# visionworkbench/visionworkbench

Measured on AMD Instinct MI355X. Metric: disparity Mpix/s, 4096x4096 pair, 7x7 SAD, +-64-px search, higher is better.
Workload: dtype u8

## Files before the change

### visionworkbench_amd/csrc/bm_sad_u8.hip

```cpp
#include <climits>
#include <cstdlib>
#include <type_traits>

#include "vwgpu_internal.h"
#include "u8_tile.h"

#ifdef VWGPU_TILE_STAMPS
__device__ unsigned long long* g_sad_stamps = nullptr;
extern "C" int vwgpu_debug_set_sad_stamps(void* d_buf) {
  unsigned long long* p = static_cast<unsigned long long*>(d_buf);
  return hipMemcpyToSymbol(HIP_SYMBOL(g_sad_stamps), &p, sizeof p) == hipSuccess ? 0 : -3;
}
#define VWGPU_STAMP(k) do { if (g_sad_stamps && tid == 0) g_sad_stamps[(size_t)wg * 16 + (k)] = wall_clock64(); } while (0)
#else
#define VWGPU_STAMP(k) do { } while (0)
#endif

namespace {

using namespace vwgpu_u8;
typedef uint32_t u32;
typedef uint64_t u64;
typedef unsigned short u16x2 __attribute__((ext_vector_type(2)));

__device__ __forceinline__ u32 pk_sub_u16(u32 a, u32 b) {
  return __builtin_bit_cast(u32, (u16x2)(__builtin_bit_cast(u16x2, a) - __builtin_bit_cast(u16x2, b)));
}
__device__ __forceinline__ u32 pk_max_u16(u32 a, u32 b) {
  return __builtin_bit_cast(u32, __builtin_elementwise_max(__builtin_bit_cast(u16x2, a), __builtin_bit_cast(u16x2, b)));
}
__device__ __forceinline__ u32 pk_min_u16(u32 a, u32 b) {
  return __builtin_bit_cast(u32, __builtin_elementwise_min(__builtin_bit_cast(u16x2, a), __builtin_bit_cast(u16x2, b)));
}
__device__ __forceinline__ void umin3_acc(u32& k, u32 a, u32 b) {
  asm volatile("v_min3_u32 %0, %0, %1, %2" : "+v"(k) : "v"(a), "v"(b));
}

template <int W>
__device__ __forceinline__ void key_sub(u32& key, u32 a, u32 b) {
  if (W == 0)
    asm volatile("v_sub_u16_sdwa %0, %1, %2 dst_sel:WORD_1 dst_unused:UNUSED_PRESERVE src0_sel:WORD_0 src1_sel:WORD_0"
                 : "+v"(key) : "v"(a), "v"(b));
  else
    asm volatile("v_sub_u16_sdwa %0, %1, %2 dst_sel:WORD_1 dst_unused:UNUSED_PRESERVE src0_sel:WORD_1 src1_sel:WORD_1"
                 : "+v"(key) : "v"(a), "v"(b));
}

template <int KX, int KY, int TY, int WV = 0>
struct Cfg {
  static constexpr int NW = (KX + 3) / 4;
  static constexpr int EW = NW <= 2 ? 2 : 4;
  static constexpr int WAVES = WV ? WV : (NW <= 2 ? 4 : 2);
  static constexpr int THREADS = WAVES * 64;
  static constexpr int TWB = WAVES * 256;
  static constexpr int NR = TY + KY - 1;
  static constexpr int LBW = TWB / 4 + NW + 1;
  static constexpr u32 LAST_MASK = (KX % 4 == 0) ? 0xffffffffu : ((1u << (8 * (KX % 4))) - 1u);
};

__device__ __forceinline__ void divmod_small(int idx, int d, float inv, int& quo, int& rem) {
  int qq = (int)(((float)idx + 0.5f) * inv);
  int rr = idx - qq * d;
  if (rr < 0) { --qq; rr += d; }
  if (rr >= d) { ++qq; rr -= d; }
  quo = qq; rem = rr;
}

__device__ __forceinline__ bool sad_second_on_cu(unsigned block, int first_round) {
  return (int)(block >> 3) >= (first_round >> 4);
}

__host__ __device__ constexpr size_t ent_words(int nr, int ne, int ew, int gr, int ty, int pt) {
  const size_t ent = (size_t)nr * ne * ew;
  const size_t merge = gr > 1 ? (size_t)(gr - 1) * (ty / gr) * 4 * pt + (size_t)gr * pt : 0;
  const size_t ob = (size_t)gr * (pt / 64) * 768;
  return ent > merge ? (ent > ob ? ent : ob) : (merge > ob ? merge : ob);
}

template <int KX, int KY, int TY, int GR, int WV = 0, bool EM = true, bool STREAM = false>
__global__ void __launch_bounds__((GR * (Cfg<KX, KY, TY, WV>::THREADS)), (GR > 1 ? 1 : (TY <= 8 && KX <= 8 ? 3 : 2)))
bm_sad_u8_kernel(const float* __restrict__ L, ptrdiff_t ls, int lw, int lh,
                 const float* __restrict__ R, ptrdiff_t rs, int rcw, int rch,
                 int sx, int sy, int ne, int32_t* __restrict__ out, ptrdiff_t os, int ow, int oh,
                 int* __restrict__ flag_set, int* __restrict__ flag_clear,
                 int gxt, int ntiles, int last_round, int first_round, int stagger_ticks) {
  typedef Cfg<KX, KY, TY, WV> C;
  constexpr bool SPLIT = GR > 1;
  static_assert(!(STREAM && SPLIT), "streaming output stores: one-group kernels only");
  constexpr int NW = C::NW, EW = C::EW, NR = C::NR;
  constexpr int NRP = EM ? (NR | 1) : NR;
  extern __shared__ __attribute__((aligned(16))) u32 lds[];
  u32* ent = lds;
  const int bpitch = ne + NW + 1;
  u32* base = lds + ent_words(NRP, ne, EW, GR, TY, C::THREADS);
  u32* item_ctr = base + (size_t)NR * bpitch;

  constexpr int PT = C::THREADS;
  constexpr int NT = GR * PT;
  const int tid = threadIdx.x;
  const int grp = SPLIT ? __builtin_amdgcn_readfirstlane(tid / PT) : 0;
  const int ltid = SPLIT ? tid % PT : tid;
  const int pair_id = __builtin_amdgcn_readfirstlane(ltid >> 6);
  const int per_xcd = gridDim.x >> 3;
  const int wg = (int)(blockIdx.x & 7) * per_xcd + (int)(blockIdx.x >> 3);
  if (wg >= ntiles) return;
  const int x0 = (wg % gxt) * C::TWB;
  const int y0 = (wg / gxt) * TY;
  const int q = x0 + 4 * ltid;
  u32 bad_acc = 0;
  if (wg == 0 && tid == 0) *flag_clear = 0;
#ifdef VWGPU_TILE_STAMPS
  if (g_sad_stamps && tid == 0) {
    unsigned hw, xcc;
    asm volatile("s_getreg_b32 %0, hwreg(HW_REG_HW_ID)" : "=s"(hw));
    asm volatile("s_getreg_b32 %0, hwreg(HW_REG_XCC_ID)" : "=s"(xcc));
    unsigned long long* rec = g_sad_stamps + (size_t)wg * 16;
    rec[0] = wall_clock64(); rec[1] = clock64(); rec[2] = ((unsigned long long)xcc << 32) | hw;
  }
#endif

  if (!SPLIT && (int)blockIdx.x < first_round && sad_second_on_cu(blockIdx.x, first_round)) {
    if (tid < 64) {
      const u64 t_start = wall_clock64();
      for (int it = 0; it < 512 && wall_clock64() - t_start < (u64)stagger_ticks; ++it) __builtin_amdgcn_s_sleep(8);
    }
    __syncthreads();
  }
  stage_u8_rows<NR>(L, ls, lw, lh, x0, y0, C::LBW, C::LBW, ent, tid, NT, bad_acc);
  stage_u8_rows<NR>(R, rs, rcw, rch, x0, y0, bpitch, bpitch, base, tid, NT, bad_acc);
  __syncthreads();
  u64 win[NR][NW];
#pragma unroll
  for (int r = 0; r < NR; ++r) {
    u32 a[NW + 1];
#pragma unroll
    for (int n = 0; n <= NW; ++n) a[n] = ent[r * C::LBW + ltid + n];
#pragma unroll
    for (int n = 0; n < NW; ++n) win[r][n] = (u64)a[n] | ((u64)a[n + 1] << 32);
  }

  VWGPU_STAMP(3);
  u32 K[TY][4];
  u32 MN[TY][2], MX[TY][2];
#pragma unroll
  for (int y = 0; y < TY; ++y) K[y][0] = K[y][1] = K[y][2] = K[y][3] = 0xffffffffu;
  u32 eq_rows = (1u << TY) - 1u;
  int eq_checks = 0;
  constexpr int NPROBE = 4;
  const u32 zero = 0;

  const bool late = !SPLIT && (int)blockIdx.x >= last_round;
  if (!SPLIT) { if (late) __builtin_amdgcn_s_setprio(2); else __builtin_amdgcn_s_setprio(3); }
  typedef std::true_type T;
  typedef std::false_type F;

  auto sweep = [&](auto max_tag) __attribute__((always_inline)) {
    constexpr bool MAXSWEEP = decltype(max_tag)::value;
    for (int dy = 0; dy < sy; ++dy) {
      __syncthreads();
      if (dy > 0 || (MAXSWEEP && sy > 1)) stage_u8_rows<NR>(R, rs, rcw, rch, x0, y0 + dy, bpitch, bpitch, base, tid, NT, bad_acc);
      for (int t = 0; t < 4; ++t) {
        const int a_last = (sx + 2 - t) >> 2;
        __syncthreads();
        if (!MAXSWEEP && !SPLIT && dy == 0 && late) {
          if (t == 2) __builtin_amdgcn_s_setprio(1);
          else if (t == 3) __builtin_amdgcn_s_setprio(0);
        }
        {
          auto build = [&](int r, int m) __attribute__((always_inline)) {
            const u32* bp = base + (size_t)r * bpitch + m;
            u32 b[NW + 1];
#pragma unroll
            for (int n = 0; n <= NW; ++n) b[n] = bp[n];
            u32 w[EW];
#pragma unroll
            for (int n = 0; n < EW; ++n) w[n] = 0;
#pragma unroll
            for (int n = 0; n < NW; ++n) w[n] = __builtin_amdgcn_alignbyte(b[n + 1], b[n], t);
            w[NW - 1] &= C::LAST_MASK;
            u32* e = ent + (EM ? (size_t)m * NRP + r : (size_t)r * ne + m) * EW;
            if (EW == 2) *reinterpret_cast<uint2*>(e) = make_uint2(w[0], w[1]);
            else *reinterpret_cast<uint4*>(e) = make_uint4(w[0], w[1], w[2 % EW], w[3 % EW]);
          };
#pragma unroll 4
          for (int r = grp; r < NR; r += NT / PT) build(r, ltid);
          const int rem = ne - PT, total = NR * rem;
          const float inv = 1.0f / (float)rem;
          for (int idx = tid; idx < total; idx += NT) {
            int r, m;
            divmod_small(idx, rem, inv, r, m);
            build(r, PT + m);
          }
          if (SPLIT && tid < PT / 64) item_ctr[tid] = 0u;
        }
        __syncthreads();

        auto step = [&](int a, auto masked_tag, auto pair_tag, auto probe_tag) __attribute__((always_inline)) {
          constexpr bool MASKED = decltype(masked_tag)::value;
          constexpr bool PAIR = decltype(pair_tag)::value;
          constexpr bool PROBE = decltype(probe_tag)::value;
          const int jbase = 4 * a + t;
          const int ibase = dy * sx + jbase;
          u32 kinA[4], kinB[4];
          u32 orA[2] = {0u, 0u};
#pragma unroll
          for (int i = 0; i < 4; ++i) {
            kinA[i] = (u32)(ibase - i) & 0xffffu;
            kinB[i] = (u32)(ibase + 4 - i) & 0xffffu;
            if (MASKED) {
              const int d = jbase - i;
              if (d < 0 || d >= sx) orA[i >> 1] |= (i & 1) ? 0xffff0000u : 0x0000ffffu;
            }
          }
          const u32* ep = ent + (size_t)(ltid + a) * (EM ? NRP * EW : EW);
          u64 accA = 0, accB = 0;
          u64 PA[NR], PB[NR];
          constexpr int PF = 4;
          u32 wa[NR][EW], wb[NR][EW];
          auto fetch = [&](int r) __attribute__((always_inline)) {
            const u32* e = ep + (EM ? (size_t)r * EW : (size_t)r * ne * EW);
            constexpr int NX = EM ? NRP * EW : EW;
            if (EW == 2) {
              const uint2 v = *reinterpret_cast<const uint2*>(e);
              wa[r][0] = v.x; wa[r][1] = v.y;
              if (PAIR) { const uint2 u = *reinterpret_cast<const uint2*>(e + NX); wb[r][0] = u.x; wb[r][1] = u.y; }
            } else {
              const uint4 v = *reinterpret_cast<const uint4*>(e);
              wa[r][0] = v.x; wa[r][1] = v.y; wa[r][2 % EW] = v.z; wa[r][3 % EW] = v.w;
              if (PAIR) { const uint4 u = *reinterpret_cast<const uint4*>(e + NX); wb[r][0] = u.x; wb[r][1] = u.y; wb[r][2 % EW] = u.z; wb[r][3 % EW] = u.w; }
            }
          };
#pragma unroll
          for (int r = 0; r < PF && r < NR; ++r) fetch(r);
#pragma unroll
          for (int r = 0; r < NR; ++r) {
            if (r + PF < NR) fetch(r + PF);
#pragma unroll
            for (int n = 0; n < NW; ++n) {
              accA = __builtin_amdgcn_qsad_pk_u16_u8(win[r][n], wa[r][n], accA);
              if (PAIR) accB = __builtin_amdgcn_qsad_pk_u16_u8(win[r][n], wb[r][n], accB);
            }
            PA[r] = accA;
            if (PAIR) PB[r] = accB;
            if (r >= KY - 1) {
              const int y = r - (KY - 1);
              const int ro = (r >= KY) ? r - KY : 0;
              const u32 nA0 = (u32)PA[r], nA1 = (u32)(PA[r] >> 32);
              const u32 oA0 = (r >= KY) ? (u32)PA[ro] : zero;
              const u32 oA1 = (r >= KY) ? (u32)(PA[ro] >> 32) : zero;
              if (MAXSWEEP) {
                const u32 sA0 = pk_sub_u16(nA0, oA0), sA1 = pk_sub_u16(nA1, oA1);
                MN[y][0] = pk_min_u16(MN[y][0], MASKED ? (sA0 | orA[0]) : sA0);
                MN[y][1] = pk_min_u16(MN[y][1], MASKED ? (sA1 | orA[1]) : sA1);
                MX[y][0] = pk_max_u16(MX[y][0], MASKED ? (sA0 & ~orA[0]) : sA0);
                MX[y][1] = pk_max_u16(MX[y][1], MASKED ? (sA1 & ~orA[1]) : sA1);
                if (PAIR) {
                  const u32 nB0 = (u32)PB[r], nB1 = (u32)(PB[r] >> 32);
                  const u32 oB0 = (r >= KY) ? (u32)PB[ro] : zero;
                  const u32 oB1 = (r >= KY) ? (u32)(PB[ro] >> 32) : zero;
                  const u32 sB0 = pk_sub_u16(nB0, oB0), sB1 = pk_sub_u16(nB1, oB1);
                  MN[y][0] = pk_min_u16(MN[y][0], sB0);
                  MN[y][1] = pk_min_u16(MN[y][1], sB1);
                  MX[y][0] = pk_max_u16(MX[y][0], sB0);
                  MX[y][1] = pk_max_u16(MX[y][1], sB1);
                }
              } else {
                key_sub<0>(kinA[0], nA0, oA0); key_sub<1>(kinA[1], nA0, oA0);
                key_sub<0>(kinA[2], nA1, oA1); key_sub<1>(kinA[3], nA1, oA1);
                if (PAIR) {
                  const u32 nB0 = (u32)PB[r], nB1 = (u32)(PB[r] >> 32);
                  const u32 oB0 = (r >= KY) ? (u32)PB[ro] : zero;
                  const u32 oB1 = (r >= KY) ? (u32)(PB[ro] >> 32) : zero;
                  key_sub<0>(kinB[0], nB0, oB0); key_sub<1>(kinB[1], nB0, oB0);
                  key_sub<0>(kinB[2], nB1, oB1); key_sub<1>(kinB[3], nB1, oB1);
                  if (PROBE) {
                    u32 x[4];
#pragma unroll
                    for (int i = 0; i < 4; ++i) {
                      asm volatile("v_xor_b32 %0, %1, %2" : "=v"(x[i]) : "v"(kinA[i]), "v"(kinB[i]));
                      x[i] = (q + i < ow) ? x[i] : 0xffffffffu;
                    }
                    const u32 m01 = x[0] < x[1] ? x[0] : x[1], m23 = x[2] < x[3] ? x[2] : x[3];
                    if ((m01 < m23 ? m01 : m23) >> 16) eq_rows &= ~(1u << y);
                  }
                  umin3_acc(K[y][0], kinA[0], kinB[0]);
                  umin3_acc(K[y][1], kinA[1], kinB[1]);
                  umin3_acc(K[y][2], kinA[2], kinB[2]);
                  umin3_acc(K[y][3], kinA[3], kinB[3]);
                } else {
                  const u32 kA0 = (MASKED && (orA[0] & 0x0000ffffu)) ? 0xffffffffu : kinA[0];
                  const u32 kA1 = (MASKED && (orA[0] & 0xffff0000u)) ? 0xffffffffu : kinA[1];
                  const u32 kA2 = (MASKED && (orA[1] & 0x0000ffffu)) ? 0xffffffffu : kinA[2];
                  const u32 kA3 = (MASKED && (orA[1] & 0xffff0000u)) ? 0xffffffffu : kinA[3];
                  umin3_acc(K[y][0], kA0, kA0);
                  umin3_acc(K[y][1], kA1, kA1);
                  umin3_acc(K[y][2], kA2, kA2);
                  umin3_acc(K[y][3], kA3, kA3);
                }
              }
            }
          }
        };

        int a_lo = (t >= 3) ? 0 : 1;
        int a_hi = (sx - 1 - t >= 0) ? ((sx - 1 - t) >> 2) + 1 : 0;
        if (a_hi > a_last + 1) a_hi = a_last + 1;
        if (a_lo > a_hi) a_lo = a_hi;
        const int n1 = a_lo;
        const int npair = (a_hi - n1) > 0 ? (a_hi - n1) >> 1 : 0;
        int nprobe = 0;
        if (!MAXSWEEP && dy == 0 && t == 0) nprobe = npair < NPROBE - eq_checks ? npair : NPROBE - eq_checks;
        const int a4 = n1 + 2 * npair;
        const int n4 = a_last - a4 + 1 > 0 ? a_last - a4 + 1 : 0;
        const int nitems = n1 + npair + n4;
        int seq = 0;
        auto next_item = [&]() __attribute__((always_inline)) -> int {
          if (MAXSWEEP) return grp == 0 ? seq++ : 0x7fffffff;
          if (!SPLIT) return seq++;
          int lane, v = 0;
          asm volatile("v_mbcnt_lo_u32_b32 %0, -1, 0\n\tv_mbcnt_hi_u32_b32 %0, -1, %0" : "=v"(lane));
          if (lane == 0) v = (int)atomicAdd(&item_ctr[pair_id], 1u);
          return __builtin_amdgcn_readfirstlane(v);
        };
        int i = next_item();
        for (; i < n1; i = next_item()) step(i, T{}, F{}, F{});
        for (; i < n1 + nprobe; i = next_item()) step(n1 + 2 * (i - n1), F{}, T{}, T{});
        for (; i < n1 + npair; i = next_item()) step(n1 + 2 * (i - n1), F{}, T{}, F{});
        for (; i < nitems; i = next_item()) step(a4 + (i - n1 - npair), T{}, F{}, F{});
        eq_checks += nprobe;
        if (!MAXSWEEP && dy == 0) VWGPU_STAMP(4 + t);
      }
    }
  };
  sweep(F{});
  if (!SPLIT) __builtin_amdgcn_s_setprio(3);

  if (bad_acc != 0u) atomicOr(flag_set, 1);
  constexpr int RG = TY / GR;
  static_assert(TY % GR == 0, "rows per group");
  auto row_mine = [&](int y) __attribute__((always_inline)) -> bool { return !SPLIT || (y / RG == grp); };
  if (SPLIT) {
    u32* xk = ent;
    u32* xe = ent + (size_t)(GR - 1) * RG * 4 * PT;
    u32 eq_all = eq_rows;
#pragma unroll
    for (int d = 0; d < GR; ++d) {
      __syncthreads();
      if (grp != d) {
        const int slot = grp < d ? grp : grp - 1;
#pragma unroll
        for (int y = 0; y < RG; ++y)
#pragma unroll
          for (int s2 = 0; s2 < 4; ++s2) xk[((slot * RG + y) * 4 + s2) * PT + ltid] = K[d * RG + y][s2];
      }
      if (d == 0) xe[grp * PT + ltid] = eq_rows;
      __syncthreads();
      if (grp == d) {
#pragma unroll
        for (int slot = 0; slot < GR - 1; ++slot)
#pragma unroll
          for (int y = 0; y < RG; ++y)
#pragma unroll
            for (int s2 = 0; s2 < 4; ++s2) {
              const u32 o = xk[((slot * RG + y) * 4 + s2) * PT + ltid];
              K[d * RG + y][s2] = o < K[d * RG + y][s2] ? o : K[d * RG + y][s2];
            }
      }
      if (d == 0) {
#pragma unroll
        for (int g2 = 0; g2 < GR; ++g2) eq_all &= xe[g2 * PT + ltid];
      }
    }
    eq_rows = eq_all;
  }
  u32 cand = eq_checks < NPROBE ? (1u << TY) - 1u : eq_rows;
#pragma unroll
  for (int y = 0; y < TY; ++y)
    if (y0 + y >= oh || q >= ow || !row_mine(y)) cand &= ~(1u << y);
  const int any = __syncthreads_or(cand != 0u);

  {
    const int wv = ltid >> 6, lane = ltid & 63;
    u32* ob = ent + (size_t)(grp * (PT / 64) + wv) * 768;
    const int xw = x0 + 256 * wv;
    int nd = (ow - xw) * 3;
    nd = nd < 0 ? 0 : (nd > 768 ? 768 : nd);
    const u32 sx_magic = sx > 1 ? (u32)(0xffffffffu / (u32)sx) + 1u : 0u;
    struct __attribute__((packed, aligned(4))) U4 { u32 x, y, z, w; };
    typedef u32 V4 __attribute__((ext_vector_type(4), aligned(4)));
    auto put = [&](u32 v, int32_t* p) __attribute__((always_inline)) {
      if constexpr (STREAM) __builtin_nontemporal_store((int32_t)v, p);
      else *p = (int32_t)v;
    };
#pragma unroll
    for (int y = 0; y < TY; ++y) {
      const int oy = y0 + y;
      if (oy >= oh || !row_mine(y)) continue;
      u32 v[12];
#pragma unroll
      for (int s = 0; s < 4; ++s) {
        const u32 di = K[y][s] & 0xffffu;
        u32 dx, dy;
        if (sy == 1) { dx = di; dy = 0; }
        else { dy = sx == 1 ? di : __umulhi(di, sx_magic); dx = di - dy * (u32)sx; }
        v[3 * s] = dx;
        v[3 * s + 1] = dy;
        v[3 * s + 2] = 0x7fffffffu;
      }
      uint4* ow4 = reinterpret_cast<uint4*>(ob + lane * 12);
      ow4[0] = make_uint4(v[0], v[1], v[2], v[3]);
      ow4[1] = make_uint4(v[4], v[5], v[6], v[7]);
      ow4[2] = make_uint4(v[8], v[9], v[10], v[11]);
      int32_t* orow = out + ((ptrdiff_t)oy * os + xw) * 3;
#pragma unroll
      for (int k = 0; k < 3; ++k) {
        const int idx = k * 256 + lane * 4;
        const uint4 t = *reinterpret_cast<const uint4*>(ob + idx);
        if (idx + 3 < nd) {
          if constexpr (STREAM) {
            const V4 u = {t.x, t.y, t.z, t.w};
            __builtin_nontemporal_store(u, reinterpret_cast<V4*>(orow + idx));
          } else {
            U4 u; u.x = t.x; u.y = t.y; u.z = t.z; u.w = t.w;
            *reinterpret_cast<U4*>(orow + idx) = u;
          }
        } else {
          if (idx < nd) put(t.x, orow + idx);
          if (idx + 1 < nd) put(t.y, orow + idx + 1);
          if (idx + 2 < nd) put(t.z, orow + idx + 2);
        }
      }
    }
  }

#ifdef VWGPU_TILE_STAMPS
  if (g_sad_stamps && tid == 0) { g_sad_stamps[(size_t)wg * 16 + 8] = wall_clock64(); g_sad_stamps[(size_t)wg * 16 + 9] = clock64(); }
#endif
  if (__builtin_expect(!any, 1)) return;
#pragma unroll
  for (int y = 0; y < TY; ++y) {
    MN[y][0] = MN[y][1] = 0xffffffffu;
    MX[y][0] = MX[y][1] = 0u;
  }
  sweep(T{});
  if (grp == 0) {
#pragma unroll
    for (int y = 0; y < TY; ++y) {
      const u32 same0 = MN[y][0] ^ MX[y][0], same1 = MN[y][1] ^ MX[y][1];
      const bool inv[4] = {(same0 & 0xffffu) == 0, (same0 >> 16) == 0, (same1 & 0xffffu) == 0, (same1 >> 16) == 0};
#pragma unroll
      for (int s = 0; s < 4; ++s)
        if (inv[s] && y0 + y < oh && q + s < ow)
          out[((ptrdiff_t)(y0 + y) * os + q + s) * 3 + 2] = 0;
    }
  }
}

typedef void (*KernelFn)(const float*, ptrdiff_t, int, int, const float*, ptrdiff_t, int, int, int, int, int,
                         int32_t*, ptrdiff_t, int, int, int*, int*, int, int, int, int, int);
struct Launch {
  int kx, ky, ty;
  int threads, twb, nr, ew, nw;
  int split_groups;
  KernelFn fn;
  KernelFn split_fn;
  KernelFn fn_rm, split_fn_rm;
  KernelFn fn_nt, fn_nt_rm;
};

template <bool ON, int KX, int KY, int TY, int GR, int WV, bool EM, bool STREAM = false>
constexpr KernelFn kernel_if() {
  if constexpr (ON) return bm_sad_u8_kernel<KX, KY, TY, GR, WV, EM, STREAM>;
  else return nullptr;
}

template <int KX, int KY, int TY, bool WITH_SPLIT = false, int WV = 0>
constexpr Launch make_launch() {
  typedef Cfg<KX, KY, TY, WV> C;
  return Launch{KX, KY, TY, C::THREADS, C::TWB, C::NR, C::EW, C::NW, WV ? 4 : 2,
                kernel_if<WV == 0, KX, KY, TY, 1, WV, true>(),
                kernel_if<WITH_SPLIT, KX, KY, TY, (WV ? 4 : 2), WV, true>(),
                kernel_if<WV == 0, KX, KY, TY, 1, WV, false>(),
                kernel_if<WITH_SPLIT, KX, KY, TY, (WV ? 4 : 2), WV, false>(),
                kernel_if<WV == 0, KX, KY, TY, 1, WV, true, true>(),
                kernel_if<WV == 0, KX, KY, TY, 1, WV, false, true>()};
}

const Launch kLaunch[] = {
    make_launch<3, 3, 16>(), make_launch<5, 5, 16>(), make_launch<7, 7, 16, true>(), make_launch<7, 7, 8, true>(), make_launch<7, 7, 16, true, 2>(),
    make_launch<7, 5, 16>(), make_launch<9, 9, 12>(), make_launch<11, 11, 8>(),
};

const Launch* find_launch(int kx, int ky) {
  for (const Launch& l : kLaunch)
    if (l.kx == kx && l.ky == ky) return &l;
  return nullptr;
}

const Launch* pick_launch(int kx, int ky, int ow, int oh, int num_cu, int groups, bool* split) {
  const Launch* best = nullptr;
  double best_cost = 0.0;
  *split = false;
  if (groups == 3) {
    bool has = false;
    for (const Launch& l : kLaunch) has |= l.kx == kx && l.ky == ky && l.split_fn && !l.fn;
    if (!has) groups = 0;
  }
  for (const Launch& l : kLaunch) {
    if (l.kx != kx || l.ky != ky) continue;
    const long long wgs = (long long)((ow + l.twb - 1) / l.twb) * ((oh + l.ty - 1) / l.ty);
    const double n = (double)((wgs + num_cu - 1) / num_cu);
    const int resident = (l.ty <= 8 && l.kx <= 8) ? 3 : 2;
    const bool narrow = l.twb * 2 <= 4 * 256 && l.split_fn && !l.fn;
    const double wfrac = narrow ? 0.5 : 1.0;
    for (int sp = 0; sp < 2; ++sp) {
      if (sp && !l.split_fn) continue;
      if (!sp && !l.fn) continue;
      if (groups == 3 && !narrow) continue;
      if (groups && groups != 3 && (narrow || (l.split_fn && (groups == 2) != (sp == 1)))) continue;
      const double steps = (sp ? l.nr * 0.55 * n : (n < 2.0 ? l.nr * 0.74 : l.nr * 0.5 * n)) * wfrac;
      const double rounds = sp ? n : (double)(((long long)n + resident - 1) / resident);
      const double cost = steps + (narrow ? 5.7 : 4.5) * rounds;
      if (!best || cost < best_cost) { best = &l; best_cost = cost; *split = sp != 0; }
    }
  }
  return best;
}

constexpr size_t kMaxLds = 80 * 1024;

constexpr int kStaggerTicks = 1400;

int entries_per_row(const Launch& l, int sx) { return l.twb / 4 + ((sx + 2) >> 2) + 1; }

size_t lds_bytes(const Launch& l, int sx, int groups, bool em) {
  const int ne = entries_per_row(l, sx);
  const size_t ent = ent_words(em ? (l.nr | 1) : l.nr, ne, l.ew, groups, l.ty, l.threads);
  const size_t left = (size_t)l.nr * (l.twb / 4 + l.nw + 1);
  const size_t base = (size_t)l.nr * (ne + l.nw + 1);
  return ((ent > left ? ent : left) + base) * sizeof(u32);
}

bool supported(const vwgpu_bm_args& a) {
  if (a.cost_type != VWGPU_ABSOLUTE_DIFFERENCE) return false;
  const Launch* l = find_launch(a.kx, a.ky);
  if (!l) return false;
  if ((long long)a.sx * a.sy > 65535) return false;
  return lds_bytes(*l, a.sx, l->split_fn ? l->split_groups : 1, false) <= kMaxLds;
}

int launch(vwgpu_ctx* ctx, const vwgpu_bm_args& a, int** d_flag) {
  const int kx = a.kx, sx = a.sx, sy = a.sy, ow = a.ow(), oh = a.oh();
  bool split = false;
  const int plan_cu = ctx->sad_round_slots > 0 ? (ctx->sad_round_slots + 1) / 2 : ctx->num_cu;
  const Launch* l = pick_launch(kx, a.ky, ow, oh, plan_cu, ctx->sad_groups, &split);
  if (!l) return vwgpu_fail(ctx, VWGPU_ERR_NOIMPL, "no packed-u8 kernel for %dx%d", kx, a.ky);
  const int rcw = a.lw + sx - 1, rch = a.lh + sy - 1;
  const int gx = (ow + l->twb - 1) / l->twb, gy = (oh + l->ty - 1) / l->ty;
  const int ne = entries_per_row(*l, sx);
  const int groups = split ? l->split_groups : 1;
  const size_t ctr_bytes = split ? 64 : 0;
  const bool em = ctx->sad_layout == 0 && lds_bytes(*l, sx, groups, true) + ctr_bytes <= kMaxLds;
  const size_t shmem = lds_bytes(*l, sx, groups, em) + ctr_bytes;
  const unsigned grid1 = (unsigned)((gx * gy + 7) / 8 * 8);
  const int resident = (l->ty <= 8 && l->kx <= 8) ? 3 : 2;
  const int slots = ctx->sad_round_slots > 0 ? ctx->sad_round_slots : ctx->num_cu * resident;
  const bool rounds = !split && (int)grid1 >= 2 * slots;
  const int last_round = rounds ? (int)grid1 - slots : INT_MAX;
  const KernelFn main_fn = em ? (split ? l->split_fn : rounds ? l->fn_nt : l->fn) : (split ? l->split_fn_rm : rounds ? l->fn_nt_rm : l->fn_rm);
  ctx->sad_last_launch = l->ty | (l->twb / 256) << 8 | groups << 12 | (em ? 1 : 0) << 16 | (rounds ? 1 : 0) << 17;
  const int first_round = (rounds && resident == 2) ? slots : 0;
  vwgpu_flag_pair f;
  int rc = vwgpu_packed_prologue(ctx, reinterpret_cast<const void*>(main_fn), shmem, d_flag, &f);
  if (rc) return rc;
  {
    vwgpu_prof_scope ps(ctx, "bm_sad_u8");
    hipLaunchKernelGGL(main_fn, dim3(grid1), dim3(split ? l->split_groups * l->threads : l->threads), shmem, ctx->stream,
                       a.left, a.ls, a.lw, a.lh, a.right, a.rs, rcw, rch, sx, sy, ne, a.out, a.os, ow, oh,
                       f.set, f.clear, gx, gx * gy, last_round, first_round, kStaggerTicks);
  }
  VWGPU_HIP(ctx, hipGetLastError());
  return VWGPU_OK;
}

}

vwgpu_bm_matcher vwgpu_bm_sad_u8 = {VWGPU_PATH_SAD_U8, 7, "packed-u8", supported, launch};
```

Baseline: 53330.

## Poison out-of-range disparities in SAD accumulators and pair the edge steps

For small-cost configurations, out-of-range disparity lanes are no longer masked per step. The accumulator is seeded with 0x8000 in those lanes and re-poisoned every KY rows, so those costs can never win. This lets the boundary (tail) items run as paired steps instead of single masked steps. The equality probe now folds the out-of-width mask into one v_xad per lane, and the probe loop stops early once a wave-wide ballot shows every row has settled. The risk is extra adds for the re-poisoning and a tail loop that calls step(a4) on every iteration, which looks wrong whenever there is more than one tail pair.

```diff
diff --git a/visionworkbench_amd/csrc/bm_sad_u8.hip b/visionworkbench_amd/csrc/bm_sad_u8.hip
--- a/visionworkbench_amd/csrc/bm_sad_u8.hip
+++ b/visionworkbench_amd/csrc/bm_sad_u8.hip
@@ -25,6 +25,9 @@
 
 __device__ __forceinline__ u32 pk_sub_u16(u32 a, u32 b) {
   return __builtin_bit_cast(u32, (u16x2)(__builtin_bit_cast(u16x2, a) - __builtin_bit_cast(u16x2, b)));
+}
+__device__ __forceinline__ u32 pk_add_u16(u32 a, u32 b) {
+  return __builtin_bit_cast(u32, (u16x2)(__builtin_bit_cast(u16x2, a) + __builtin_bit_cast(u16x2, b)));
 }
 __device__ __forceinline__ u32 pk_max_u16(u32 a, u32 b) {
   return __builtin_bit_cast(u32, __builtin_elementwise_max(__builtin_bit_cast(u16x2, a), __builtin_bit_cast(u16x2, b)));
@@ -153,6 +156,15 @@
   if (!SPLIT) { if (late) __builtin_amdgcn_s_setprio(2); else __builtin_amdgcn_s_setprio(3); }
   typedef std::true_type T;
   typedef std::false_type F;
+  typedef std::integral_constant<int, 0> E0;
+  typedef std::integral_constant<int, 1> E1;
+  typedef std::integral_constant<int, 2> E2;
+  constexpr bool SMALLCOST = 4 * NW * KY * 255 < 0x8000;
+  constexpr bool POISON = SMALLCOST, XPROBE = SMALLCOST && !(GR == 1 && TY <= 8 && KX <= 8);
+  auto wave_settled = [&]() __attribute__((always_inline)) -> bool {
+    const u32 rows_in = oh - y0 >= TY ? (1u << TY) - 1u : (1u << (oh - y0)) - 1u;
+    return __builtin_amdgcn_ballot_w64((eq_rows & rows_in) != 0u && q < ow) == 0ull;
+  };
 
   auto sweep = [&](auto max_tag) __attribute__((always_inline)) {
     constexpr bool MAXSWEEP = decltype(max_tag)::value;
@@ -195,25 +207,39 @@
         }
         __syncthreads();
 
-        auto step = [&](int a, auto masked_tag, auto pair_tag, auto probe_tag) __attribute__((always_inline)) {
-          constexpr bool MASKED = decltype(masked_tag)::value;
+        auto step = [&](int a, auto end_tag, auto pair_tag, auto probe_tag) __attribute__((always_inline)) {
+          constexpr bool MASKED = decltype(end_tag)::value == 1;
+          constexpr bool POISONED = decltype(end_tag)::value == 2;
           constexpr bool PAIR = decltype(pair_tag)::value;
           constexpr bool PROBE = decltype(probe_tag)::value;
+          static_assert(!POISONED || (POISON && !MAXSWEEP), "poisoned steps: the matcher sweep of the sizes the guard admits");
           const int jbase = 4 * a + t;
           const int ibase = dy * sx + jbase;
           u32 kinA[4], kinB[4];
           u32 orA[2] = {0u, 0u};
+          u32 zA[2] = {0u, 0u}, zB[2] = {0u, 0u};
 #pragma unroll
           for (int i = 0; i < 4; ++i) {
             kinA[i] = (u32)(ibase - i) & 0xffffu;
             kinB[i] = (u32)(ibase + 4 - i) & 0xffffu;
+            const int d = jbase - i;
             if (MASKED) {
-              const int d = jbase - i;
               if (d < 0 || d >= sx) orA[i >> 1] |= (i & 1) ? 0xffff0000u : 0x0000ffffu;
             }
+            if (POISONED) {
+              if (d < 0 || d >= sx) zA[i >> 1] |= (i & 1) ? 0x80000000u : 0x00008000u;
+              if (PAIR && (d + 4 < 0 || d + 4 >= sx)) zB[i >> 1] |= (i & 1) ? 0x80000000u : 0x00008000u;
+            }
+          }
+          u32 pm[4] = {0u, 0u, 0u, 0u};
+          if (PROBE && XPROBE) {
+            int ow_s = ow;
+            asm volatile("" : "+s"(ow_s));
+#pragma unroll
+            for (int i = 0; i < 4; ++i) pm[i] = (i < ow_s - q) ? 0u : 0x40000000u;
           }
           const u32* ep = ent + (size_t)(ltid + a) * (EM ? NRP * EW : EW);
-          u64 accA = 0, accB = 0;
+          u64 accA = (u64)zA[0] | ((u64)zA[1] << 32), accB = (u64)zB[0] | ((u64)zB[1] << 32);
           u64 PA[NR], PB[NR];
           constexpr int PF = 4;
           u32 wa[NR][EW], wb[NR][EW];
@@ -235,6 +261,10 @@
 #pragma unroll
           for (int r = 0; r < NR; ++r) {
             if (r + PF < NR) fetch(r + PF);
+            if (POISONED && r > 0 && r % KY == 0) {
+              accA = (u64)pk_add_u16((u32)accA, zA[0]) | ((u64)pk_add_u16((u32)(accA >> 32), zA[1]) << 32);
+              if (PAIR) accB = (u64)pk_add_u16((u32)accB, zB[0]) | ((u64)pk_add_u16((u32)(accB >> 32), zB[1]) << 32);
+            }
 #pragma unroll
             for (int n = 0; n < NW; ++n) {
               accA = __builtin_amdgcn_qsad_pk_u16_u8(win[r][n], wa[r][n], accA);
@@ -275,13 +305,21 @@
                   key_sub<0>(kinB[2], nB1, oB1); key_sub<1>(kinB[3], nB1, oB1);
                   if (PROBE) {
                     u32 x[4];
-#pragma unroll
-                    for (int i = 0; i < 4; ++i) {
-                      asm volatile("v_xor_b32 %0, %1, %2" : "=v"(x[i]) : "v"(kinA[i]), "v"(kinB[i]));
-                      x[i] = (q + i < ow) ? x[i] : 0xffffffffu;
+                    if (XPROBE) {
+#pragma unroll
+                      for (int i = 0; i < 4; ++i)
+                        asm volatile("v_xad_u32 %0, %1, %2, %3" : "=v"(x[i]) : "v"(kinA[i]), "v"(kinB[i]), "v"(pm[i]));
+                      const u32 m01 = x[0] < x[1] ? x[0] : x[1], m012 = m01 < x[2] ? m01 : x[2];
+                      if ((m012 < x[3] ? m012 : x[3]) >> 16) eq_rows &= ~(1u << y);
+                    } else {
+#pragma unroll
+                      for (int i = 0; i < 4; ++i) {
+                        asm volatile("v_xor_b32 %0, %1, %2" : "=v"(x[i]) : "v"(kinA[i]), "v"(kinB[i]));
+                        x[i] = (q + i < ow) ? x[i] : 0xffffffffu;
+                      }
+                      const u32 m01 = x[0] < x[1] ? x[0] : x[1], m23 = x[2] < x[3] ? x[2] : x[3];
+                      if ((m01 < m23 ? m01 : m23) >> 16) eq_rows &= ~(1u << y);
                     }
-                    const u32 m01 = x[0] < x[1] ? x[0] : x[1], m23 = x[2] < x[3] ? x[2] : x[3];
-                    if ((m01 < m23 ? m01 : m23) >> 16) eq_rows &= ~(1u << y);
                   }
                   umin3_acc(K[y][0], kinA[0], kinB[0]);
                   umin3_acc(K[y][1], kinA[1], kinB[1]);
@@ -322,11 +360,23 @@
           if (lane == 0) v = (int)atomicAdd(&item_ctr[pair_id], 1u);
           return __builtin_amdgcn_readfirstlane(v);
         };
+        constexpr bool PZ = POISON && !MAXSWEEP;
+        typedef std::conditional_t<PZ, E2, E1> EE;
         int i = next_item();
-        for (; i < n1; i = next_item()) step(i, T{}, F{}, F{});
-        for (; i < n1 + nprobe; i = next_item()) step(n1 + 2 * (i - n1), F{}, T{}, T{});
-        for (; i < n1 + npair; i = next_item()) step(n1 + 2 * (i - n1), F{}, T{}, F{});
-        for (; i < nitems; i = next_item()) step(a4 + (i - n1 - npair), T{}, F{}, F{});
+        bool settled = false;
+        for (; i < n1; i = next_item()) step(i, EE{}, F{}, F{});
+        for (; i < n1 + nprobe && !settled; i = next_item()) {
+          step(n1 + 2 * (i - n1), E0{}, T{}, T{});
+          if (!MAXSWEEP && XPROBE) settled = wave_settled();
+        }
+        for (; i < n1 + npair; i = next_item()) step(n1 + 2 * (i - n1), E0{}, T{}, F{});
+        if constexpr (PZ) {
+          const int nend = n4 >> 1;
+          for (; i < n1 + npair + nend; i = next_item()) step(a4, E2{}, T{}, F{});
+          for (; i < n1 + npair + nend + (n4 & 1); i = next_item()) step(a4 + 2 * nend, E2{}, F{}, F{});
+        } else {
+          for (; i < nitems; i = next_item()) step(a4 + (i - n1 - npair), E1{}, F{}, F{});
+        }
         eq_checks += nprobe;
         if (!MAXSWEEP && dy == 0) VWGPU_STAMP(4 + t);
       }
```

New measurement: 54160, median of 6. 1.02x the previous value.
